# XDzzzzzZyq/b-pinn-kalman-filter

Hardware: AMD Instinct MI355X
Metric: PC-sampler score-net evals/s (NCSN++ 128x128x1, EM + Langevin) (higher is better)
Workload: dtype f32; 1 GPU; configs[2]: NCSN++ 128x128x1 PC sampler, VP-SDE N=1000, euler_maruyama + langevin (snr 0.075), global batch 64 = 64/GPU x 1; model=ncsnpp (62.69M params), global_batch=64, per_gpu_batch=64, parallelism=dp1 (batch-sharded, RCCL), hip_graph=True, pc_graph_allreduce=False

## Files before the change

b-pinn-kalman-filter_amd/csrc/conv_winograd.hip:

```cpp
#include "bpk_common.h"
#include "wino_f24.h"

#include <algorithm>
#include <cstdlib>
#include <type_traits>

namespace {

using f4 = __attribute__((ext_vector_type(4))) float;

constexpr int kTR = 4, kTC = 8;
constexpr int kM = kTR * kTC;
constexpr int kPR = 2 * kTR + 2;
constexpr int kPC = 2 * kTC + 2;
constexpr int kPCp = 24;
constexpr int kCK = 8;
constexpr int kOutRows = 2 * kTR, kOutCols = 2 * kTC;

__device__ inline void wino_filter_range(const float* __restrict__ w, float* __restrict__ U,
                                         int Cin, int Cout, int CoutP, int ft, int64_t first,
                                         int64_t stride) {
  const int64_t total = (int64_t)Cin * CoutP;
  for (int64_t i = first; i < total; i += stride) {
    const int co = (int)(i % CoutP);
    const int ci = (int)(i / CoutP);
    if (co >= Cout) {
      f4* u = reinterpret_cast<f4*>(U + ((int64_t)ci * CoutP + co) * 16);
#pragma unroll
      for (int r = 0; r < 4; ++r) u[r] = f4{0.f, 0.f, 0.f, 0.f};
      continue;
    }
    const float* g = ft ? w + ((int64_t)ci * Cout + co) * 9 : w + ((int64_t)co * Cin + ci) * 9;
    auto gv = [&](int k) { return ft ? g[8 - k] : g[k]; };
    float t[4][3];
#pragma unroll
    for (int c = 0; c < 3; ++c) {
      const float g0 = gv(c), g1 = gv(3 + c), g2 = gv(6 + c);
      t[0][c] = g0;
      t[1][c] = 0.5f * (g0 + g1 + g2);
      t[2][c] = 0.5f * (g0 - g1 + g2);
      t[3][c] = g2;
    }
    float* u = U + ((int64_t)ci * CoutP + co) * 16;
#pragma unroll
    for (int r = 0; r < 4; ++r) {
      const float a0 = t[r][0], a1 = t[r][1], a2 = t[r][2];
      u[4 * r + 0] = a0;
      u[4 * r + 1] = 0.5f * (a0 + a1 + a2);
      u[4 * r + 2] = 0.5f * (a0 - a1 + a2);
      u[4 * r + 3] = a2;
    }
  }
}

__global__ __launch_bounds__(256) void wino_filter_kernel(const float* __restrict__ w,
                                                          float* __restrict__ U, int Cin,
                                                          int Cout, int CoutP, int ft) {
  wino_filter_range(w, U, Cin, Cout, CoutP, ft, (int64_t)blockIdx.x * blockDim.x + threadIdx.x,
                    (int64_t)gridDim.x * blockDim.x);
}

__global__ __launch_bounds__(256) void wino_filter_batch_kernel(const int64_t* __restrict__ jobs) {
  const int64_t* jb = jobs + 6 * (int64_t)blockIdx.y;
  wino_filter_range(reinterpret_cast<const float*>(jb[0]), reinterpret_cast<float*>(jb[1]),
                    (int)jb[2], (int)jb[3], (int)jb[4], (int)jb[5],
                    (int64_t)blockIdx.x * blockDim.x + threadIdx.x,
                    (int64_t)gridDim.x * blockDim.x);
}

__global__ __launch_bounds__(256) void wino_filter24_kernel(const float* __restrict__ w,
                                                            float* __restrict__ U, int Cin,
                                                            int Cout, int CoutP, int ft) {
  const int64_t total = (int64_t)Cin * CoutP;
  for (int64_t i = (int64_t)blockIdx.x * blockDim.x + threadIdx.x; i < total;
       i += (int64_t)gridDim.x * blockDim.x) {
    const int co = (int)(i % CoutP);
    const int ci = (int)(i / CoutP);
    float u[24];
    if (co >= Cout) {
#pragma unroll
      for (int p = 0; p < 24; ++p) u[p] = 0.f;
    } else {
      const float* g = ft ? w + ((int64_t)ci * Cout + co) * 9 : w + ((int64_t)co * Cin + ci) * 9;
      float gg[9];
#pragma unroll
      for (int k = 0; k < 9; ++k) gg[k] = ft ? g[8 - k] : g[k];
      wino24_filter(gg, u);
    }
    f4* dst = reinterpret_cast<f4*>(U) + ((int64_t)ci * (CoutP / 16) + co / 16) * 96 + co % 16;
#pragma unroll
    for (int q = 0; q < 6; ++q)
      dst[16 * q] = f4{u[4 * q], u[4 * q + 1], u[4 * q + 2], u[4 * q + 3]};
  }
}

struct WinoGeo {
  int N, Cin, Cout, H, W;
  int regions_x, regions_y, cout_blocks;
  float div;
  int C1;
  int CoutS;
  int up;
  int ksplit;
  int pair;
};

constexpr int kVS = 20;
constexpr int kPreMaxCin = 1024;


__device__ inline float silu_f(float z) { return z * __builtin_amdgcn_rcpf(1.f + __expf(-z)); }

__device__ inline unsigned udivmod(unsigned a, unsigned d, unsigned& r) {
  if ((d & (d - 1)) == 0) {
    r = a & (d - 1);
    return a >> __builtin_ctz(d);
  }
  const unsigned q = a / d;
  r = a - q * d;
  return q;
}

__device__ inline float div_rn(float a, float b, float r) {
  const float q = a * r;
  return fmaf(fmaf(-q, b, a), r, q);
}

template <int CTRL>
__device__ inline float dpp_f(float v) {
  return __int_as_float(__builtin_amdgcn_mov_dpp(__float_as_int(v), CTRL, 0xF, 0xF, false));
}

__device__ inline void merge_stats(float& m, float& m2, float mo, float m2o, float c) {
  const float d = mo - m;
  m2 = (m2 + m2o) + d * d * (0.5f * c);
  m = 0.5f * (m + mo);
}

#ifdef WINO_TIMING
constexpr unsigned kTsMax = 1u << 17;
__device__ long long g_wino_ts[kTsMax][8];
__device__ unsigned g_wino_cu[kTsMax];
#define WINO_TS_AT(rec, slot)                                                      \
  do {                                                                             \
    if (threadIdx.x == 0 && (rec) < kTsMax) {                                      \
      g_wino_ts[rec][slot] = wall_clock64();                                       \
      if (slot == 0) g_wino_cu[rec] = __smid();                                    \
      if (slot == 0 || slot == 5)                                                  \
        g_wino_ts[rec][6 + slot / 5] = (long long)__builtin_amdgcn_s_memtime();    \
    }                                                                              \
  } while (0)
#else
#define WINO_TS_AT(rec, slot) \
  do {                        \
  } while (0)
#endif
#define WINO_TS(slot) WINO_TS_AT(blockIdx.x, slot)

template <bool PRE, int WG = 4, bool TAIL = false>
__global__ __launch_bounds__(64 * WG, WG == 8 ? 1 : 2) void wino_f23_pipe_kernel(
    const float* __restrict__ x, const float* __restrict__ U, const float* __restrict__ bias,
    const float* __restrict__ skip, const float2* __restrict__ pre, float* __restrict__ y,
    float2* __restrict__ stats, WinoGeo g, int xcd_remap, const float* __restrict__ x2) {
  constexpr int kWN = 16;
  constexpr int kPatch = kCK * kPR * kPCp;
  __shared__ __attribute__((aligned(16))) float s_patch_raw[2][kPatch];
  constexpr int kVBuf = kCK * kM * kVS;
  __shared__ __attribute__((aligned(16))) float s_v[2][kVBuf];
  __shared__ float2 s_ss[PRE ? kPreMaxCin : 1];

  WINO_TS(0);
  const int tid = threadIdx.x;
  const int wave = tid >> 6, lane = tid & 63;
  const unsigned nblk = gridDim.x;
  unsigned b = blockIdx.x;
  if (xcd_remap) b = (b & 7u) * (nblk >> 3) + (b >> 3);
  unsigned cb, rx, ry;
  unsigned r = udivmod(b, (unsigned)g.cout_blocks, cb);
  r = udivmod(r, (unsigned)g.regions_x, rx);
  const int n = (int)udivmod(r, (unsigned)g.regions_y, ry);
  const int oy0 = (int)ry * kOutRows, ox0 = (int)rx * kOutCols;
  const int cout_w = (int)cb * (WG * kWN) + wave * kWN;
  constexpr int kCT = kCK * 4 / WG;
  const int phc = WG == 8 ? __builtin_amdgcn_readfirstlane(tid >> 8) : 0;

  f4 acc[16][2];

  const int64_t plane = (int64_t)g.H * g.W;
  const int C2 = g.Cin - g.C1;
  const float* xn = x + (int64_t)n * g.C1 * plane;
  const float2* pre_n = PRE ? pre + (int64_t)n * g.Cin : nullptr;
  const int kq = lane >> 4, jj = lane & 15;
  const int nch = g.Cin / kCK;

  const __amdgpu_buffer_rsrc_t xrs = __builtin_amdgcn_make_buffer_rsrc(
      const_cast<float*>(xn), 0, (int)(g.C1 * plane * 4), 0x00020000);
  const __amdgpu_buffer_rsrc_t xrs2 = __builtin_amdgcn_make_buffer_rsrc(
      const_cast<float*>(C2 > 0 ? x2 + (int64_t)n * C2 * plane : xn), 0,
      (int)((C2 > 0 ? C2 : g.C1) * plane * 4), 0x00020000);
  const __amdgpu_buffer_rsrc_t urs = __builtin_amdgcn_make_buffer_rsrc(
      const_cast<float*>(U), 0, (int)((int64_t)g.Cin * g.Cout * 64), 0x00020000);

  constexpr int kPos = kPR * kPC;
  int poff, pdst;
  bool pin;
  {
    const int t8 = tid & 255;
    const int t = t8 < kPos ? t8 : 0;
    const int py = t / kPC, px = t - py * kPC;
    const int iy = oy0 - 1 + py, ix = ox0 - 1 + px;
    pin = iy >= 0 && iy < g.H && ix >= 0 && ix < g.W;
    const int cy = min(max(iy, 0), g.H - 1), cx = min(max(ix, 0), g.W - 1);
    poff = (cy * g.W + cx) * 4;
    pdst = py * kPCp + px + phc * kCT * (kPR * kPCp);
  }
  float pv[kCT];
  auto load_patch = [&](int k) {
    const int cc = min(k, nch - 1) * kCK;
    const bool second = cc >= g.C1;
    const int soff = ((second ? cc - g.C1 : cc) + phc * kCT) * (int)plane * 4;
#pragma unroll
    for (int c = 0; c < kCT; ++c)
      pv[c] = __uint_as_float(__builtin_amdgcn_raw_buffer_load_b32(
          second ? xrs2 : xrs, poff, soff + c * (int)plane * 4, 0));
  };
  auto store_patch_from = [&](const float* src, float* sp, int k) {
    const int c0 = min(k, nch - 1) * kCK + phc * kCT;
#pragma unroll
    for (int c = 0; c < kCT; ++c) {
      float v = src[c];
      if (PRE) {
        const float2 st = s_ss[c0 + c];
        v = silu_f(v * st.x + st.y);
      }
      sp[pdst + c * (kPR * kPCp)] = pin ? v : 0.f;
    }
  };
  auto store_patch = [&](float* sp, int k) { store_patch_from(pv, sp, k); };
  f4 uo[2][4];
  const int uoff = ((kq * g.Cout + cout_w + jj) * 16) * 4;
  auto load_u = [&](int ks, int k) {
    const int soff = ((min(k, nch - 1) * kCK + 4 * ks) * g.Cout) * 64;
#pragma unroll
    for (int q = 0; q < 4; ++q) {
      using u4 = __attribute__((ext_vector_type(4))) unsigned;
      const u4 w = __builtin_amdgcn_raw_buffer_load_b128(urs, uoff + q * 16, soff, 0);
      uo[ks][q] = __builtin_bit_cast(f4, w);
    }
  };
  const int tc = (tid & 255) >> 5, tm = tid & 31;
  const int tty = tm / kTC, ttx = tm - tty * kTC;
  float d[4][4];
  auto read_d = [&](const float* sp) {
#pragma unroll
    for (int i = 0; i < 4; ++i)
#pragma unroll
      for (int j = 0; j < 4; j += 2) {
        const float2 v2 =
            *reinterpret_cast<const float2*>(&sp[(tc * kPR + 2 * tty + i) * kPCp + 2 * ttx + j]);
        d[i][j] = v2.x;
        d[i][j + 1] = v2.y;
      }
  };
  auto write_v = [&](float* sv) {
    float t[4][4];
#pragma unroll
    for (int j = 0; j < 4; ++j) {
      t[0][j] = d[0][j] - d[2][j];
      t[1][j] = d[1][j] + d[2][j];
      t[2][j] = d[2][j] - d[1][j];
      t[3][j] = d[1][j] - d[3][j];
    }
    f4* dst = reinterpret_cast<f4*>(&sv[(tc * kM + tm) * kVS]);
#pragma unroll
    for (int i = 0; i < 4; ++i)
      dst[i] = f4{t[i][0] - t[i][2], t[i][1] + t[i][2], t[i][2] - t[i][1], t[i][1] - t[i][3]};
  };

  float pv0[kCT], pv1[kCT];
  load_patch(0);
#pragma unroll
  for (int c = 0; c < kCT; ++c) pv0[c] = pv[c];
  load_patch(1);
#pragma unroll
  for (int c = 0; c < kCT; ++c) pv1[c] = pv[c];
  load_patch(2);
  load_u(0, 0);
  load_u(1, 0);
  if (PRE) {
    for (int c = tid; c < g.Cin; c += 64 * WG) s_ss[c] = pre_n[c];
    __syncthreads();
  }
  WINO_TS(1);
  store_patch_from(pv0, s_patch_raw[0], 0);
  store_patch_from(pv1, s_patch_raw[1], 1);
  __syncthreads();
  WINO_TS(2);
  read_d(s_patch_raw[0]);
  write_v(s_v[0]);
  __syncthreads();

  f4 a[4];
  auto a_src = [&](const float* sv, int grp) {
    const int ks = grp >> 1, mb = grp & 1;
    return reinterpret_cast<const f4*>(&sv[((4 * ks + kq) * kM + mb * 16 + jj) * kVS]);
  };
  {
    const f4* src = a_src(s_v[0], 0);
#pragma unroll
    for (int q = 0; q < 4; ++q) a[q] = src[q];
  }
  auto step = [&](int k, auto sb_c, auto first_c, auto tm_c) __attribute__((always_inline)) {
    constexpr int SB = decltype(sb_c)::value;
    constexpr bool FIRST = decltype(first_c)::value;
    constexpr int TM = decltype(tm_c)::value;
    const float* sv = s_v[SB];
#pragma unroll
    for (int grp = 0; grp < 4; ++grp) {
      const int ks = grp >> 1, mb = grp & 1;
      __builtin_amdgcn_sched_barrier(0);
      if (TM < 3 && grp == 0) read_d(s_patch_raw[SB ^ 1]);
      if (TM < 3 && grp == 1) write_v(s_v[SB ^ 1]);
      if (TM < 2 && grp == 2) store_patch(s_patch_raw[SB], k + 2);
      if (TM < 1 && grp == 3) load_patch(k + 3);
      __builtin_amdgcn_sched_barrier(0);
#pragma unroll
      for (int q = 0; q < 4; ++q) {
#pragma unroll
        for (int pp = 0; pp < 4; ++pp)
          acc[4 * q + pp][mb] = __builtin_amdgcn_mfma_f32_16x16x4f32(
              a[q][pp], uo[ks][q][pp],
              (FIRST && ks == 0) ? f4{0.f, 0.f, 0.f, 0.f} : acc[4 * q + pp][mb], 0, 0, 0);
        if (grp < 3) a[q] = a_src(sv, grp + 1)[q];
        if (TM < 3 && mb == 1) {
          const int soff = ((min(k + 1, nch - 1) * kCK + 4 * ks) * g.Cout) * 64;
          using u4 = __attribute__((ext_vector_type(4))) unsigned;
          const u4 w = __builtin_amdgcn_raw_buffer_load_b128(urs, uoff + q * 16, soff, 0);
          uo[ks][q] = __builtin_bit_cast(f4, w);
        }
      }
    }
    if constexpr (TM < 3) {
      __syncthreads();
      const f4* src = a_src(s_v[SB ^ 1], 0);
#pragma unroll
      for (int q = 0; q < 4; ++q) a[q] = src[q];
    }
  };
  using C0 = std::integral_constant<int, 0>;
  using C1 = std::integral_constant<int, 1>;
  using F = std::false_type;
  WINO_TS(3);
  using T0 = std::integral_constant<int, 0>;
  auto run = [&]() __attribute__((always_inline)) {
    step(0, C0{}, std::true_type{}, T0{});
    int k = 1;
    if constexpr (TAIL) {
      for (; k + 1 <= nch - 4; k += 2) {
        step(k, C1{}, F{}, T0{});
        step(k + 1, C0{}, F{}, T0{});
      }
      step(k, C1{}, F{}, std::integral_constant<int, 1>{});
      step(k + 1, C0{}, F{}, std::integral_constant<int, 2>{});
      step(k + 2, C1{}, F{}, std::integral_constant<int, 3>{});
    } else {
      for (; k + 1 < nch; k += 2) {
        step(k, C1{}, F{}, T0{});
        step(k + 1, C0{}, F{}, T0{});
      }
      if (k < nch) step(k, C1{}, F{}, T0{});
    }
  };
  run();
  WINO_TS(4);

  const float rdiv = 1.f / g.div;
  for (int once = 0; once < 1; ++once) {
    if (cout_w >= g.CoutS) continue;
    const int co = cout_w + jj;
    const float bv = bias ? bias[co] : 0.f;
    const int64_t obase = ((int64_t)n * g.CoutS + co) * plane;
    float lm = 0.f, lm2 = 0.f;
#pragma unroll
    for (int mb = 0; mb < 2; ++mb) {
      const int oy = oy0 + 2 * (2 * mb + (kq >> 1));
      const int ox = ox0 + 8 * (kq & 1);
#pragma unroll
      for (int h = 0; h < 2; ++h) {
#pragma unroll
        for (int e = 0; e < 2; ++e) {
          f4 v;
#pragma unroll
          for (int u = 0; u < 2; ++u) {
            const int rg = 2 * e + u;
            float t[4];
#pragma unroll
            for (int j = 0; j < 4; ++j)
              t[j] = h == 0 ? acc[j][mb][rg] + acc[4 + j][mb][rg] + acc[8 + j][mb][rg]
                            : acc[4 + j][mb][rg] - acc[8 + j][mb][rg] - acc[12 + j][mb][rg];
            v[2 * u] = t[0] + t[1] + t[2] + bv;
            v[2 * u + 1] = t[1] - t[2] - t[3] + bv;
          }
          const int64_t o = obase + (int64_t)(oy + h) * g.W + ox + 4 * e;
          if (skip) {
            const f4 sk = *reinterpret_cast<const f4*>(&skip[o]);
#pragma unroll
            for (int c = 0; c < 4; ++c) v[c] = div_rn(sk[c] + v[c], g.div, rdiv);
          }
          *reinterpret_cast<f4*>(&y[o]) = v;
          if (stats) {
            const float sm = ((v[0] + v[1]) + (v[2] + v[3])) * 0.25f;
            float sm2 = 0.f;
#pragma unroll
            for (int c = 0; c < 4; ++c) sm2 = fmaf(v[c] - sm, v[c] - sm, sm2);
            constexpr float kW[8] = {1.f, 1.f / 2, 1.f / 3, 1.f / 4, 1.f / 5, 1.f / 6, 1.f / 7, 1.f / 8};
            const int st = 4 * mb + 2 * h + e;
            const float d = sm - lm;
            lm = lm + d * kW[st];
            lm2 = (lm2 + sm2) + d * d * (4.f * st * kW[st]);
          }
        }
      }
    }
    if (stats) {
      merge_stats(lm, lm2, __shfl_xor(lm, 16, 64), __shfl_xor(lm2, 16, 64), 32.f);
      merge_stats(lm, lm2, __shfl_xor(lm, 32, 64), __shfl_xor(lm2, 32, 64), 64.f);
      if (kq == 0) {
        const int R = g.regions_x * g.regions_y;
        const int region = (oy0 / kOutRows) * g.regions_x + ox0 / kOutCols;
        stats[((int64_t)n * g.CoutS + co) * R + region] = make_float2(lm, lm2);
      }
    }
  }
  WINO_TS(5);
}

template <bool PRE, bool PAIR>
__device__ __forceinline__ void k16_item(
    unsigned b, const float* __restrict__ x, const float* __restrict__ U,
// ... 208 lines not shown
    const float bv = bias ? bias[co] : 0.f;
    const int oimg = PAIR ? n + (kq & 1) : n;
    const int oxl = PAIR ? 0 : ox0 + 8 * (kq & 1);
    const int64_t obase = ((int64_t)(ks_idx * g.N + oimg) * g.CoutS + co) * plane;
    float lm = 0.f, lm2 = 0.f;
    f4 skv[2][2][2];
    if (skip) {
#pragma unroll
      for (int mb = 0; mb < 2; ++mb)
#pragma unroll
        for (int h = 0; h < 2; ++h)
#pragma unroll
          for (int e = 0; e < 2; ++e)
            skv[mb][h][e] = *reinterpret_cast<const f4*>(
                &skip[obase + (int64_t)(oy0 + 2 * (2 * mb + (kq >> 1)) + h) * g.W + oxl + 4 * e]);
    }
#pragma unroll
    for (int mb = 0; mb < 2; ++mb) {
      const int oy = oy0 + 2 * (2 * mb + (kq >> 1));
      const int ox = oxl;
#pragma unroll
      for (int h = 0; h < 2; ++h) {
#pragma unroll
        for (int e = 0; e < 2; ++e) {
          f4 v;
#pragma unroll
          for (int u = 0; u < 2; ++u) {
            const int rg = 2 * e + u;
            float t[4];
#pragma unroll
            for (int j = 0; j < 4; ++j)
              t[j] = h == 0 ? acc[j][mb][rg] + acc[4 + j][mb][rg] + acc[8 + j][mb][rg]
                            : acc[4 + j][mb][rg] - acc[8 + j][mb][rg] - acc[12 + j][mb][rg];
            v[2 * u] = t[0] + t[1] + t[2] + bv;
            v[2 * u + 1] = t[1] - t[2] - t[3] + bv;
          }
          const int64_t o = obase + (int64_t)(oy + h) * g.W + ox + 4 * e;
          if (skip) {
            const f4 sk = skv[mb][h][e];
#pragma unroll
            for (int c = 0; c < 4; ++c) v[c] = div_rn(sk[c] + v[c], g.div, rdiv);
          }
          *reinterpret_cast<f4*>(&y[o]) = v;
          if (!PAIR && stats) {
            const float sm = ((v[0] + v[1]) + (v[2] + v[3])) * 0.25f;
            float sm2 = 0.f;
#pragma unroll
            for (int c = 0; c < 4; ++c) sm2 = fmaf(v[c] - sm, v[c] - sm, sm2);
            constexpr float kW[8] = {1.f, 1.f / 2, 1.f / 3, 1.f / 4, 1.f / 5, 1.f / 6, 1.f / 7, 1.f / 8};
            const int st = 4 * mb + 2 * h + e;
            const float dd = sm - lm;
            lm = lm + dd * kW[st];
            lm2 = (lm2 + sm2) + dd * dd * (4.f * st * kW[st]);
          }
        }
      }
    }
    if (!PAIR && stats) {
      merge_stats(lm, lm2, __shfl_xor(lm, 16, 64), __shfl_xor(lm2, 16, 64), 32.f);
      merge_stats(lm, lm2, __shfl_xor(lm, 32, 64), __shfl_xor(lm2, 32, 64), 64.f);
      if (kq == 0) {
        const int R = g.regions_x * g.regions_y;
        const int region = (oy0 / kOutRows) * g.regions_x + ox0 / kOutCols;
        stats[((int64_t)n * g.CoutS + co) * R + region] = make_float2(lm, lm2);
      }
    }
  }
  WINO_TS(5);
}

template <bool PRE, bool PAIR = false>
__global__ __launch_bounds__(512, 1) void wino_f23_k16_kernel(
    const float* __restrict__ x, const float* __restrict__ U, const float* __restrict__ bias,
    const float* __restrict__ skip, const float2* __restrict__ pre, float* __restrict__ y,
    float2* __restrict__ stats, WinoGeo g, int xcd_remap, const float* __restrict__ x2,
    unsigned items) {
  const unsigned G = gridDim.x, w = blockIdx.x;
  unsigned first = w, stride = G, end = items;
  if (xcd_remap) {
    const unsigned xc = w & 7u, q = items >> 3, r = items & 7u;
    const unsigned start = xc * q + min(xc, r);
    first = start + (w >> 3);
    stride = G >> 3;
    end = start + q + (xc < r ? 1u : 0u);
  }
  for (unsigned b = first; b < end; b += stride) {
    if (b != first) __syncthreads();
    k16_item<PRE, PAIR>(b, x, U, bias, skip, pre, y, stats, g, x2);
  }
}

constexpr int kM24 = 16;
constexpr int kVS24 = 28;

struct Item24Carry {
  f4 uo[2][6];
  int tab_n;
  bool u_ready;
};

template <bool PRE, bool TAILK>
__device__ __forceinline__ void k16_item24(
    unsigned b, unsigned nb, const float* __restrict__ x, const float* __restrict__ U,
    const float* __restrict__ bias, const float* __restrict__ skip,
    const float2* __restrict__ pre, float* __restrict__ y, float2* __restrict__ stats,
    const WinoGeo& g, const float* __restrict__ x2, Item24Carry& carry) {
  constexpr int kOob = (int)0x80000000u;
  constexpr int CK = 16;
  constexpr int kPatch = CK * kPR * kPCp;
  __shared__ __attribute__((aligned(16))) float s_patch_raw[2][kPatch];
  constexpr int kVBuf = CK * kM24 * kVS24;
  __shared__ __attribute__((aligned(16))) float s_v[2][kVBuf];
  __shared__ float2 s_ss[PRE ? kPreMaxCin : 1];

  const int tid = threadIdx.x;
  const int wave = tid >> 6, lane = tid & 63;
  unsigned cb, rx, ry;
  unsigned r = udivmod(b, (unsigned)g.cout_blocks, cb);
  r = udivmod(r, (unsigned)g.regions_x, rx);
  r = udivmod(r, (unsigned)g.regions_y, ry);
  unsigned nn;
  const int ks_idx = (int)udivmod(r, (unsigned)g.N, nn);
  const int n = (int)nn;
  const int oy0 = (int)ry * kOutRows, ox0 = (int)rx * kOutCols;
  const int cout_w = (int)cb * 128 + wave * 16;
  const int ph = __builtin_amdgcn_readfirstlane(tid >> 8);
  WINO_TS_AT(b, 0);
  bool u_next = false;
  if (TAILK && nb != ~0u) {
    unsigned cb2, t2;
    unsigned r2 = udivmod(nb, (unsigned)g.cout_blocks, cb2);
    r2 = udivmod(r2, (unsigned)g.regions_x, t2);
    r2 = udivmod(r2, (unsigned)g.regions_y, t2);
    u_next = cb2 == cb && (int)udivmod(r2, (unsigned)g.N, t2) == ks_idx;
  }

  f4 acc[24];
  const int64_t plane = (int64_t)g.H * g.W;
  const int up = g.up;
  const int64_t xplane = plane >> (2 * up);
  const int C2 = g.Cin - g.C1;
  const float* xn = x + (int64_t)n * g.C1 * xplane;
  const float2* pre_n = PRE ? pre + (int64_t)n * g.Cin : nullptr;
  const int kq = lane >> 4, jj = lane & 15;
  const int nch = g.Cin / CK / max(g.ksplit, 1);
  const int kb = ks_idx * nch;

  const __amdgpu_buffer_rsrc_t xrs = __builtin_amdgcn_make_buffer_rsrc(
      const_cast<float*>(xn), 0, (int)(g.C1 * xplane * 4), 0x00020000);
  const __amdgpu_buffer_rsrc_t xrs2 = __builtin_amdgcn_make_buffer_rsrc(
      const_cast<float*>(C2 > 0 ? x2 + (int64_t)n * C2 * plane : xn), 0,
      (int)((C2 > 0 ? C2 : g.C1) * plane * 4), 0x00020000);
  const __amdgpu_buffer_rsrc_t urs = __builtin_amdgcn_make_buffer_rsrc(
      const_cast<float*>(U), 0, (int)((int64_t)g.Cin * g.Cout * 96), 0x00020000);

  constexpr int kPos = kPR * kPC;
  int poff, pdst;
  bool pin;
  {
    const int t8 = tid & 255;
    const int t = t8 < kPos ? t8 : 0;
    const int py = t / kPC, px = t - py * kPC;
    const int iy = oy0 - 1 + py, ix = ox0 - 1 + px;
    pin = iy >= 0 && iy < g.H && ix >= 0 && ix < g.W;
    const int cy = min(max(iy, 0), g.H - 1), cx = min(max(ix, 0), g.W - 1);
    poff = ((cy >> up) * (g.W >> up) + (cx >> up)) * 4;
    pdst = py * kPCp + px + ph * 8 * (kPR * kPCp);
  }
  float pv[8];
  auto load_patch_part = [&](float* dst, int k, int c0, int cn, bool guard = false) {
    const int cc = (kb + min(k, nch - 1)) * CK;
    const bool second = cc >= g.C1;
    const int soff = ((second ? cc - g.C1 : cc) + ph * 8) * (int)xplane * 4;
    const int po = (guard && k >= nch) ? kOob : poff;
#pragma unroll
    for (int c = c0; c < c0 + cn; ++c)
      dst[c] = __uint_as_float(__builtin_amdgcn_raw_buffer_load_b32(
          second ? xrs2 : xrs, po, soff + c * (int)xplane * 4, 0));
  };
  auto store_patch_part = [&](const float* src, float* sp, int k, int c0, int cn) {
    const int cb0 = (kb + min(k, nch - 1)) * CK + ph * 8;
#pragma unroll
    for (int c = c0; c < c0 + cn; ++c) {
      float v = src[c];
      if (PRE) {
        const float2 st = s_ss[cb0 + c];
        v = silu_f(v * st.x + st.y);
      }
      sp[pdst + c * (kPR * kPCp)] = pin ? v : 0.f;
    }
  };
  f4(&uo)[2][6] = carry.uo;
  const int uoff = ((kq * g.Cout + cout_w) * 24 + jj * 4) * 4;
  auto u_soff = [&](int k, int ks) {
    return (((kb + min(k, nch - 1)) * CK + 4 * ks) * g.Cout) * 96;
  };
  const int u_soff0[2] = {__builtin_amdgcn_readfirstlane(u_soff(0, 0)),
                          __builtin_amdgcn_readfirstlane(u_soff(0, 1))};
  auto load_u = [&](int slot, int k, int ks) {
    const int soff = u_soff(k, ks);
#pragma unroll
    for (int q = 0; q < 6; ++q)
      uo[slot][q] = __builtin_bit_cast(
          f4, __builtin_amdgcn_raw_buffer_load_b128(urs, uoff + q * 256, soff, 0));
  };
  const int th = __builtin_amdgcn_readfirstlane(wave & 1);
  const int tc = 4 * kq + (wave >> 1);
  const int tty = jj >> 2, ttx = jj & 3;
  float d[3][6];
  auto read_d = [&](const float* sp) {
#pragma unroll
    for (int i = 0; i < 3; ++i) {
      const float* row = &sp[(tc * kPR + 2 * tty + th + i) * kPCp + 4 * ttx];
      const f4 v4 = *reinterpret_cast<const f4*>(row);
      const float2 v2 = *reinterpret_cast<const float2*>(row + 4);
      d[i][0] = v4[0];
      d[i][1] = v4[1];
      d[i][2] = v4[2];
      d[i][3] = v4[3];
      d[i][4] = v2.x;
      d[i][5] = v2.y;
    }
  };
  auto write_v = [&](float* sv) {
    float rx_[6], ry_[6], vx[6], vy[6];
#pragma unroll
    for (int j = 0; j < 6; ++j) wino24_data_rows(d[0][j], d[1][j], d[2][j], th, rx_[j], ry_[j]);
    wino24_data_cols(rx_, vx);
    wino24_data_cols(ry_, vy);
    f4* dst = reinterpret_cast<f4*>(&sv[(tc * kM24 + jj) * kVS24 + 12 * th]);
    dst[0] = f4{vx[0], vx[1], vx[2], vx[3]};
    dst[1] = f4{vx[4], vx[5], vy[0], vy[1]};
    dst[2] = f4{vy[2], vy[3], vy[4], vy[5]};
  };

  const bool tab_load = PRE && carry.tab_n != n;
  const bool u_have = TAILK && carry.u_ready;
  carry.tab_n = n;
  carry.u_ready = u_next;
  {
    float pv0[8], pv1[8];
    float2 tv[kPreMaxCin / 512];
    if (tab_load) {
#pragma unroll
      for (int i = 0; i < kPreMaxCin / 512; ++i) tv[i] = pre_n[min(tid + 512 * i, g.Cin - 1)];
    }
    __builtin_amdgcn_sched_barrier(0);
    load_patch_part(pv0, 0, 0, 8);
    __builtin_amdgcn_sched_barrier(0);
    load_patch_part(pv1, 1, 0, 8, TAILK);
    load_patch_part(pv, 2, 0, 8, TAILK);
    if (!u_have) {
      load_u(0, 0, 0);
      load_u(1, 0, 1);
    }
    __builtin_amdgcn_sched_barrier(0);
    if (tab_load) {
#pragma unroll
      for (int i = 0; i < kPreMaxCin / 512; ++i)
        if (tid + 512 * i < g.Cin) s_ss[tid + 512 * i] = tv[i];
      __syncthreads();
    }
    store_patch_part(pv0, s_patch_raw[0], 0, 0, 8);
    __syncthreads();
    read_d(s_patch_raw[0]);
    write_v(s_v[0]);
    if (!TAILK || nch > 1) store_patch_part(pv1, s_patch_raw[1], 1, 0, 8);
  }
  __syncthreads();
  WINO_TS_AT(b, 1);

  f4 a[4];
  auto a_src = [&](const float* sv, int ks) {
    return reinterpret_cast<const f4*>(&sv[((4 * ks + kq) * kM24 + jj) * kVS24]);
  };
  {
    const f4* src = a_src(s_v[0], 0);
#pragma unroll
    for (int q = 0; q < 4; ++q) a[q] = src[q];
  }
  auto step = [&](int k, auto sb_c, auto first_c, auto tail_c) __attribute__((always_inline)) {
    constexpr int SB = decltype(sb_c)::value;
    constexpr bool FIRST = decltype(first_c)::value;
    constexpr int TL = decltype(tail_c)::value;
    const float* sv = s_v[SB];
#pragma unroll
    for (int grp = 0; grp < 8; ++grp) {
      const int ks = grp >> 1, hf = grp & 1;
      __builtin_amdgcn_sched_barrier(0);
      if (grp == 0 && TL < 3) read_d(s_patch_raw[SB ^ 1]);
      if (grp == 1 && TL < 3) write_v(s_v[SB ^ 1]);
      if (grp == 2 && TL < 2) store_patch_part(pv, s_patch_raw[SB], k + 2, 0, 4);
      if (grp == 3 && TL < 2) store_patch_part(pv, s_patch_raw[SB], k + 2, 4, 4);
      if (grp == 4 && TL < 1) load_patch_part(pv, k + 3, 0, 4);
      if (grp == 5 && TL < 1) load_patch_part(pv, k + 3, 4, 4);
      __builtin_amdgcn_sched_barrier(0);
#pragma unroll
      for (int qq = 0; qq < 3; ++qq) {
        const int q = 3 * hf + qq;
        const int fi = 6 * ks + q;
#pragma unroll
        for (int pp = 0; pp < 4; ++pp)
          acc[4 * q + pp] = __builtin_amdgcn_mfma_f32_16x16x4f32(
              a[fi & 3][pp], uo[ks & 1][q][pp],
              (FIRST && ks == 0) ? f4{0.f, 0.f, 0.f, 0.f} : acc[4 * q + pp], 0, 0, 0);
        if (fi + 4 < 24) a[fi & 3] = a_src(sv, (fi + 4) / 6)[(fi + 4) % 6];
        if (ks < 2 || TL < 3 || TAILK) {
          const int soff = ks < 2 ? u_soff(k, ks + 2)
                                  : (TL < 3 ? u_soff(k + 1, ks - 2) : u_soff0[ks - 2]);
          uo[ks & 1][q] = __builtin_bit_cast(
              f4, __builtin_amdgcn_raw_buffer_load_b128(urs, uoff + q * 256, soff, 0));
        }
      }
    }
    if (TL < 3) {
      __syncthreads();
      const f4* src = a_src(s_v[SB ^ 1], 0);
#pragma unroll
      for (int q = 0; q < 4; ++q) a[q] = src[q];
    }
  };
  using C0 = std::integral_constant<int, 0>;
  using C1 = std::integral_constant<int, 1>;
  using T2 = std::integral_constant<int, 2>;
  using T3 = std::integral_constant<int, 3>;
  using Fi = std::true_type;
  using No = std::false_type;
  WINO_TS_AT(b, 2);
  if (!TAILK) {
    step(0, C0{}, Fi{}, C0{});
    int k = 1;
    for (; k + 1 < nch; k += 2) {
      step(k, C1{}, No{}, C0{});
      step(k + 1, C0{}, No{}, C0{});
    }
    if (k < nch) step(k, C1{}, No{}, C0{});
  } else {
    if (nch >= 4) {
      step(0, C0{}, Fi{}, C0{});
      int k = 1;
      for (; k + 3 < nch; k += 2) {
        step(k, C1{}, No{}, C0{});
        step(k + 1, C0{}, No{}, C0{});
      }
    } else {
#pragma unroll
      for (int i = 0; i < 24; ++i) acc[i] = f4{0.f, 0.f, 0.f, 0.f};
    }
    if (nch >= 4) step(nch - 3, C1{}, No{}, C1{});
    step(nch - 2, C0{}, No{}, T2{});
    step(nch - 1, C1{}, No{}, T3{});
  }
  WINO_TS_AT(b, 3);

  const float rdiv = 1.f / g.div;
  if (cout_w < g.CoutS) {
    const int co = cout_w + jj;
    const float bv = bias ? bias[co] : 0.f;
    const int64_t obase = ((int64_t)(ks_idx * g.N + n) * g.CoutS + co) * plane +
                          (int64_t)(oy0 + 2 * kq) * g.W + ox0;
    float lm = 0.f, lm2 = 0.f;
    f4 skv[2][4];
    if (skip) {
#pragma unroll
      for (int h = 0; h < 2; ++h)
#pragma unroll
        for (int rg = 0; rg < 4; ++rg)
          skv[h][rg] = *reinterpret_cast<const f4*>(&skip[obase + (int64_t)h * g.W + 4 * rg]);
    }
#pragma unroll
    for (int h = 0; h < 2; ++h) {
#pragma unroll
      for (int rg = 0; rg < 4; ++rg) {
        float t[6], yv[4];
#pragma unroll
        for (int j = 0; j < 6; ++j)
          t[j] = wino24_out_rows(acc[j][rg], acc[6 + j][rg], acc[12 + j][rg], acc[18 + j][rg], h);
        wino24_out_cols(t, yv);
        f4 v = f4{yv[0] + bv, yv[1] + bv, yv[2] + bv, yv[3] + bv};
        const int64_t o = obase + (int64_t)h * g.W + 4 * rg;
        if (skip) {
          const f4 sk = skv[h][rg];
#pragma unroll
          for (int c = 0; c < 4; ++c) v[c] = div_rn(sk[c] + v[c], g.div, rdiv);
        }
        *reinterpret_cast<f4*>(&y[o]) = v;
        if (stats) {
          const float sm = ((v[0] + v[1]) + (v[2] + v[3])) * 0.25f;
          float sm2 = 0.f;
#pragma unroll
          for (int c = 0; c < 4; ++c) sm2 = fmaf(v[c] - sm, v[c] - sm, sm2);
          constexpr float kW[8] = {1.f, 1.f / 2, 1.f / 3, 1.f / 4, 1.f / 5, 1.f / 6, 1.f / 7, 1.f / 8};
          const int st = 4 * h + rg;
          const float dd = sm - lm;
          lm = lm + dd * kW[st];
          lm2 = (lm2 + sm2) + dd * dd * (4.f * st * kW[st]);
        }
      }
    }
    WINO_TS_AT(b, 4);
    if (stats) {
      merge_stats(lm, lm2, __shfl_xor(lm, 16, 64), __shfl_xor(lm2, 16, 64), 32.f);
      merge_stats(lm, lm2, __shfl_xor(lm, 32, 64), __shfl_xor(lm2, 32, 64), 64.f);
      if (kq == 0) {
        const int R = g.regions_x * g.regions_y;
        const int region = (oy0 / kOutRows) * g.regions_x + ox0 / kOutCols;
        stats[((int64_t)n * g.CoutS + co) * R + region] = make_float2(lm, lm2);
      }
    }
  }
  WINO_TS_AT(b, 5);
}

template <bool PRE, bool TAILK>
__global__ __launch_bounds__(512, 1) void wino_f24_k16_kernel(
    const float* __restrict__ x, const float* __restrict__ U, const float* __restrict__ bias,
    const float* __restrict__ skip, const float2* __restrict__ pre, float* __restrict__ y,
    float2* __restrict__ stats, WinoGeo g, int xcd_remap, const float* __restrict__ x2,
    unsigned items) {
  const unsigned G = gridDim.x, w = blockIdx.x;
  unsigned first = w, stride = G, end = items;
  if (xcd_remap) {
    const unsigned xc = w & 7u, q = items >> 3, r = items & 7u;
    const unsigned start = xc * q + min(xc, r);
    first = start + (w >> 3);
    stride = G >> 3;
    end = start + q + (xc < r ? 1u : 0u);
  }
  Item24Carry carry;
  carry.tab_n = -1;
  carry.u_ready = false;
  for (unsigned b = first; b < end; b += stride) {
    if (b != first) __syncthreads();
    const unsigned nb = b + stride < end ? b + stride : ~0u;
    k16_item24<PRE, TAILK>(b, nb, x, U, bias, skip, pre, y, stats, g, x2, carry);
  }
}

__global__ __launch_bounds__(256) void wino_splitk_reduce_kernel(
    const float* __restrict__ part, int S, const float* __restrict__ bias,
    const float* __restrict__ skip, float* __restrict__ y, float2* __restrict__ stats,
    WinoGeo g) {
  const int lane = threadIdx.x & 63;
  const int q = threadIdx.x;
  unsigned b = blockIdx.x, reg, cg;
  const unsigned R = (unsigned)(g.regions_x * g.regions_y);
  unsigned r = udivmod(b, R, reg);
  int n = (int)udivmod(r, (unsigned)(g.CoutS / 8), cg);
  const int co = (int)cg * 8 + (q >> 5);
  const int rem = q & 31;
  const int row = rem >> 2;
  int c4 = rem & 3;
  if (g.pair) {
    n = 2 * n + (c4 >> 1);
    c4 &= 1;
  }
  const int oy0 = (int)(reg / g.regions_x) * kOutRows, ox0 = (int)(reg % g.regions_x) * kOutCols;
  const int64_t plane = (int64_t)g.H * g.W;
  const int64_t slab = (int64_t)g.N * g.CoutS * plane;
  const int64_t o = ((int64_t)n * g.CoutS + co) * plane + (int64_t)(oy0 + row) * g.W + ox0 + 4 * c4;
  f4 v = *reinterpret_cast<const f4*>(&part[o]);
  for (int s = 1; s < S; ++s) v += *reinterpret_cast<const f4*>(&part[s * slab + o]);
  const float bv = bias ? bias[co] : 0.f;
  v += f4{bv, bv, bv, bv};
  if (skip) {
    const f4 sk = *reinterpret_cast<const f4*>(&skip[o]);
    const float rdiv = 1.f / g.div;
#pragma unroll
    for (int c = 0; c < 4; ++c) v[c] = div_rn(sk[c] + v[c], g.div, rdiv);
  }
  *reinterpret_cast<f4*>(&y[o]) = v;
  if (!stats || g.pair) return;
  float mm = ((v[0] + v[1]) + (v[2] + v[3])) * 0.25f;
  float qq = 0.f;
#pragma unroll
  for (int e = 0; e < 4; ++e) qq = fmaf(v[e] - mm, v[e] - mm, qq);
  merge_stats(mm, qq, dpp_f<0xB1>(mm), dpp_f<0xB1>(qq), 4.f);
  merge_stats(mm, qq, dpp_f<0x4E>(mm), dpp_f<0x4E>(qq), 8.f);
  merge_stats(mm, qq, dpp_f<0x141>(mm), dpp_f<0x141>(qq), 16.f);
  merge_stats(mm, qq, dpp_f<0x140>(mm), dpp_f<0x140>(qq), 32.f);
  merge_stats(mm, qq, __shfl_xor(mm, 16, 64), __shfl_xor(qq, 16, 64), 64.f);
  if ((lane & 31) == 0) stats[((int64_t)n * g.CoutS + co) * R + reg] = make_float2(mm, qq);
}

}

static int cout_padded(int Cout) { return (Cout + 63) / 64 * 64; }

static int cu_count() {
  static const int cus = [] {
    int dev = 0, n = 0;
    (void)hipGetDevice(&dev);
    (void)hipDeviceGetAttribute(&n, hipDeviceAttributeMultiprocessorCount, dev);
    return n > 0 ? n : 256;
  }();
  return cus;
}


extern "C" int64_t bpk_conv3x3_wino_filter_bytes(int Cin, int Cout) {
  return (int64_t)16 * Cin * cout_padded(Cout) * (int64_t)sizeof(float);
}

extern "C" int64_t bpk_conv3x3_wino_filter24_bytes(int Cin, int Cout) {
  return (int64_t)24 * Cin * cout_padded(Cout) * (int64_t)sizeof(float);
}

using FilterKernel = void (*)(const float*, float*, int, int, int, int);

static int wino_filter(FilterKernel kern, const float* weight, float* U, int Cin, int Cout,
                       int ft, void* stream) {
  BPK_REQUIRE(Cin > 0 && Cout > 0, "conv3x3_wino_filter: bad channels %d -> %d", Cin, Cout);
  const int64_t total = (int64_t)Cin * cout_padded(Cout);
  hipLaunchKernelGGL(kern, dim3((unsigned)std::min<int64_t>(bpk::ceil_div(total, 256), 4096)),
                     dim3(256), 0, bpk::as_stream(stream), weight, U, Cin, Cout,
                     cout_padded(Cout), ft);
  BPK_LAUNCH_CHECK("conv3x3_wino_filter");
  return BPK_OK;
}

extern "C" int bpk_conv3x3_wino_filter_f32(const float* weight, float* U, int Cin, int Cout,
                                           void* stream) {
  return wino_filter(wino_filter_kernel, weight, U, Cin, Cout, 0, stream);
}

extern "C" int bpk_conv3x3_wino_filter_ft_f32(const float* weight, float* U, int Cin, int Cout,
                                              void* stream) {
  return wino_filter(wino_filter_kernel, weight, U, Cin, Cout, 1, stream);
}

extern "C" int bpk_conv3x3_wino_filter24_f32(const float* weight, float* U, int Cin, int Cout,
                                             void* stream) {
  return wino_filter(wino_filter24_kernel, weight, U, Cin, Cout, 0, stream);
}

extern "C" int bpk_conv3x3_wino_filter24_ft_f32(const float* weight, float* U, int Cin, int Cout,
                                                void* stream) {
  return wino_filter(wino_filter24_kernel, weight, U, Cin, Cout, 1, stream);
}

extern "C" int bpk_conv3x3_wino_filter_batch_f32(const int64_t* jobs, int n, int max_elems,
                                                 void* stream) {
  BPK_REQUIRE(n >= 0 && n < 65536 && max_elems >= 0, "conv3x3_wino_filter_batch: bad job count");
  if (n == 0 || max_elems == 0) return BPK_OK;
  BPK_REQUIRE(jobs != nullptr, "conv3x3_wino_filter_batch: jobs is NULL");
  const dim3 grid((unsigned)std::min<int64_t>(bpk::ceil_div(max_elems, 256), 64), (unsigned)n);
  hipLaunchKernelGGL(wino_filter_batch_kernel, grid, dim3(256), 0, bpk::as_stream(stream), jobs);
  BPK_LAUNCH_CHECK("conv3x3_wino_filter_batch");
  return BPK_OK;
}


extern "C" int bpk_conv3x3_wino_supported(int N, int Cin, int Cout, int H, int W) {
  return N > 0 && Cin > 0 && Cin % kCK == 0 && Cout % 16 == 0 && H % kOutRows == 0 &&
         W % kOutCols == 0;
}

static bool k16_channels_ok(int Cin, int C1, int Cout) {
  return Cin % 16 == 0 && C1 % 16 == 0 && cout_padded(Cout) % 128 == 0;
}

static bool wino_pair_ok(int N, int Cin, int Cout, int H, int W) {
  return N > 0 && N % 2 == 0 && W == 8 && H > 0 && H % kOutRows == 0 && Cout % 16 == 0 &&
         k16_channels_ok(Cin, Cin, Cout);
}

extern "C" int bpk_conv3x3_wino_pair_supported(int N, int Cin, int Cout, int H, int W) {
  return wino_pair_ok(N, Cin, Cout, H, W);
}

extern "C" int bpk_conv3x3_wino_up2_supported(int N, int Cin, int Cout, int H, int W) {
  return bpk_conv3x3_wino_supported(N, Cin, Cout, H, W) && k16_channels_ok(Cin, Cin, Cout);
}

extern "C" int bpk_conv3x3_wino_f24_supported(int N, int Cin, int C1, int Cout, int H, int W) {
  return N > 0 && Cin > 0 && Cin <= kPreMaxCin && C1 > 0 && C1 <= Cin && Cout > 0 &&
         Cout % 16 == 0 && k16_channels_ok(Cin, C1, Cout) && H > 0 && H % kOutRows == 0 && W > 0 &&
         W % kOutCols == 0;
}


struct WinoArgs {
  const float *x, *x2, *pre, *U, *bias, *skip;
  float *y, *stats;
  void* stream;
};

static WinoGeo k16_geo(int N, int Cin, int C1, int Cout, int H, int W, float div, int up, int S,
                       int pair) {
  const int CoutP = cout_padded(Cout);
  WinoGeo g{};
  g.N = N, g.Cin = Cin, g.C1 = C1, g.Cout = CoutP, g.CoutS = Cout, g.H = H, g.W = W;
  g.regions_x = pair ? 1 : W / kOutCols;
  g.regions_y = H / kOutRows;
  g.cout_blocks = CoutP / 128;
  g.div = div, g.up = up, g.ksplit = S, g.pair = pair;
  return g;
}

static int64_t k16_items(const WinoGeo& g) {
  return (int64_t)(g.pair ? g.N / 2 : g.N) * g.regions_x * g.regions_y * g.cout_blocks * g.ksplit;
}

using K16Kernel = void (*)(const float*, const float*, const float*, const float*, const float2*,
                           float*, float2*, WinoGeo, int, const float*, unsigned);

static int k16_launch(bool f24, const WinoGeo& g, const WinoArgs& a) {
  const int64_t items = k16_items(g);
  BPK_REQUIRE(items < (1LL << 31), "conv3x3_wino: grid too large");
  static const K16Kernel kKern[2][2][2] = {
      {{wino_f23_k16_kernel<false, false>, wino_f23_k16_kernel<false, true>},
       {wino_f23_k16_kernel<true, false>, wino_f23_k16_kernel<true, true>}},
      {{wino_f24_k16_kernel<false, false>, wino_f24_k16_kernel<false, true>},
       {wino_f24_k16_kernel<true, false>, wino_f24_k16_kernel<true, true>}}};
  const bool even = (g.Cin / 16 / g.ksplit) % 2 == 0;
  const unsigned grid = (unsigned)std::min<int64_t>(items, cu_count());
  const bool raw = g.ksplit > 1;
  hipLaunchKernelGGL(kKern[f24][a.pre != nullptr][f24 ? even : g.pair != 0], dim3(grid), dim3(512),
                     0, bpk::as_stream(a.stream), a.x, a.U, raw ? nullptr : a.bias,
                     raw ? nullptr : a.skip, reinterpret_cast<const float2*>(a.pre), a.y,
                     raw ? nullptr : reinterpret_cast<float2*>(a.stats), g, grid % 8 == 0 ? 1 : 0,
                     a.x2, (unsigned)items);
  BPK_LAUNCH_CHECK(f24 ? "conv3x3_wino_f24" : "conv3x3_wino_k16");
  return BPK_OK;
}

static int wino_f24_check(int N, int Cin, int C1, int Cout, int H, int W) {
  BPK_REQUIRE(bpk_conv3x3_wino_f24_supported(N, Cin, C1, Cout, H, W),
              "conv3x3_wino_f24: unsupported shape N=%d Cin=%d (C1=%d) Cout=%d H=%d W=%d (need "
              "Cin, C1 %% 16, Cout %% 128, H %% 8, W %% 16 == 0, Cin <= %d)", N, Cin, C1, Cout, H,
              W, kPreMaxCin);
  return BPK_OK;
}

static int wino_pair_check(const WinoArgs& a, int N, int Cin, int Cout, int H, int W) {
  BPK_REQUIRE(!a.x2 && !a.stats, "conv3x3_wino pair form (W == 8): one source, no statistics");
  BPK_REQUIRE(wino_pair_ok(N, Cin, Cout, H, W),
              "conv3x3_wino pair form: unsupported shape N=%d Cin=%d Cout=%d H=%d W=%d (need "
              "W == 8, N even, H %% 8, Cin %% 16, Cout %% 128 == 0)", N, Cin, Cout, H, W);
  BPK_REQUIRE(!a.pre || 2 * Cin <= kPreMaxCin, "conv3x3_wino pair form: GroupNorm prologue over "
              "%d > %d channels", Cin, kPreMaxCin / 2);
  return BPK_OK;
}

using PipeKernel = void (*)(const float*, const float*, const float*, const float*, const float2*,
                            float*, float2*, WinoGeo, int, const float*);

static int wino_ex(const WinoArgs& a, int C1, float div, int N, int Cin, int Cout, int H, int W) {
  if (!a.x2) C1 = Cin;
  if (W == 8) {
    const int rc = wino_pair_check(a, N, Cin, Cout, H, W);
    return rc != BPK_OK ? rc : k16_launch(false, k16_geo(N, Cin, Cin, Cout, H, W, div, 0, 1, 1), a);
  }
  BPK_REQUIRE(C1 > 0 && C1 <= Cin && C1 % kCK == 0,
              "conv3x3_wino: bad channel split C1=%d of Cin=%d", C1, Cin);
  BPK_REQUIRE(bpk_conv3x3_wino_supported(N, Cin, Cout, H, W),
              "conv3x3_wino: unsupported shape N=%d Cin=%d Cout=%d H=%d W=%d (need Cin %% 8, "
              "Cout %% 16, H %% 8, W %% 16 == 0)", N, Cin, Cout, H, W);
  BPK_REQUIRE(!a.pre || Cin <= kPreMaxCin,
              "conv3x3_wino: GroupNorm prologue over %d > %d input channels (the table in LDS): "
              "apply it to the input first", Cin, kPreMaxCin);
  if (k16_channels_ok(Cin, C1, Cout))
    return k16_launch(false, k16_geo(N, Cin, C1, Cout, H, W, div, 0, 1, 0), a);
  const int CoutP = cout_padded(Cout);
  const bool wg8 = a.pre && !a.skip && CoutP % 128 == 0;
  WinoGeo g{};
  g.N = N, g.Cin = Cin, g.C1 = C1, g.Cout = CoutP, g.CoutS = Cout, g.H = H, g.W = W;
  g.regions_x = W / kOutCols, g.regions_y = H / kOutRows, g.cout_blocks = CoutP / (wg8 ? 128 : 64);
  g.div = div;
  const int64_t blocks = (int64_t)N * g.regions_x * g.regions_y * g.cout_blocks;
  BPK_REQUIRE(blocks < (1LL << 31), "conv3x3_wino: grid too large");
  const int nch = Cin / kCK;
  const bool tail = a.pre && nch % 2 == 0 && nch >= 4;
  static const PipeKernel kPipe[2][2][2] = {
      {{wino_f23_pipe_kernel<false, 4, false>, wino_f23_pipe_kernel<false, 4, false>},
       {wino_f23_pipe_kernel<false, 8, false>, wino_f23_pipe_kernel<false, 8, false>}},
      {{wino_f23_pipe_kernel<true, 4, false>, wino_f23_pipe_kernel<true, 4, true>},
       {wino_f23_pipe_kernel<true, 8, false>, wino_f23_pipe_kernel<true, 8, true>}}};
  hipLaunchKernelGGL(kPipe[a.pre != nullptr][wg8][tail], dim3((unsigned)blocks),
                     dim3(wg8 ? 512 : 256), 0, bpk::as_stream(a.stream), a.x, a.U, a.bias, a.skip,
                     reinterpret_cast<const float2*>(a.pre), a.y,
                     reinterpret_cast<float2*>(a.stats), g, blocks % 8 == 0 ? 1 : 0, a.x2);
  BPK_LAUNCH_CHECK("conv3x3_wino_pipe");
  return BPK_OK;
}

extern "C" int bpk_conv3x3_wino_ex_f32(const float* x, const float* x2, int C1, const float* pre,
                                       const float* U, const float* bias, const float* skip,
                                       float div, float* y, float* stats, int N, int Cin,
                                       int Cout, int H, int W, void* stream) {
  return wino_ex({x, x2, pre, U, bias, skip, y, stats, stream}, C1, div, N, Cin, Cout, H, W);
}

extern "C" int bpk_conv3x3_wino_pre_f32(const float* x, const float* pre, const float* U,
                                        const float* bias, const float* skip, float div, float* y,
                                        int N, int Cin, int Cout, int H, int W, void* stream) {
  return wino_ex({x, nullptr, pre, U, bias, skip, y, nullptr, stream}, Cin, div, N, Cin, Cout, H,
                 W);
}

extern "C" int bpk_conv3x3_wino_residual_f32(const float* x, const float* U, const float* bias,
                                             const float* skip, float div, float* y, int N,
                                             int Cin, int Cout, int H, int W, void* stream) {
  return bpk_conv3x3_wino_pre_f32(x, nullptr, U, bias, skip, div, y, N, Cin, Cout, H, W, stream);
}

extern "C" int bpk_conv3x3_wino_f32(const float* x, const float* U, const float* bias, float* y,
                                    int N, int Cin, int Cout, int H, int W, void* stream) {
  return bpk_conv3x3_wino_pre_f32(x, nullptr, U, bias, nullptr, 1.0f, y, N, Cin, Cout, H, W,
                                  stream);
// ... 95 lines not shown
```

Baseline: 827.3 score-net evals/s.

## Transpose MFMA operands in Winograd F24 k16 epilogue to change output lane mapping

Swaps the A/B operands of the 16x16x4 MFMA so the accumulator layout puts output channels across lanes differently, then rewrites the epilogue to index by four channels per lane with per-row spatial tiles, loading bias as a vector and computing per-channel stats via quad DPP transposes plus shuffles. The aim is to change the store and skip-load access pattern and the stats reduction cost. It relies on new lane variables (tty, ttx) and changes which channel each lane writes, so correctness depends on the rest of the kernel defining them consistently. It also adds an optional debug macro path that collapses the stores into one.

Measured after the change: 853.9 score-net evals/s, median of 6. +3.2%, better.

```diff
diff --git a/b-pinn-kalman-filter_amd/csrc/conv_winograd.hip b/b-pinn-kalman-filter_amd/csrc/conv_winograd.hip
--- a/b-pinn-kalman-filter_amd/csrc/conv_winograd.hip
+++ b/b-pinn-kalman-filter_amd/csrc/conv_winograd.hip
@@ -135,6 +135,19 @@
   const float d = mo - m;
   m2 = (m2 + m2o) + d * d * (0.5f * c);
   m = 0.5f * (m + mo);
+}
+
+template <int CTRL>
+__device__ inline void quad_swap(float& lo, float& hi, bool upper) {
+  const float plo = dpp_f<CTRL>(lo), phi = dpp_f<CTRL>(hi);
+  lo = upper ? phi : lo;
+  hi = upper ? hi : plo;
+}
+__device__ inline void quad_transpose(float (&a)[4], int t) {
+  quad_swap<0xB1>(a[0], a[1], t & 1);
+  quad_swap<0xB1>(a[2], a[3], t & 1);
+  quad_swap<0x4E>(a[0], a[2], t & 2);
+  quad_swap<0x4E>(a[1], a[3], t & 2);
 }
 
 #ifdef WINO_TIMING
@@ -949,7 +962,7 @@
 #pragma unroll
         for (int pp = 0; pp < 4; ++pp)
           acc[4 * q + pp] = __builtin_amdgcn_mfma_f32_16x16x4f32(
-              a[fi & 3][pp], uo[ks & 1][q][pp],
+              uo[ks & 1][q][pp], a[fi & 3][pp],
               (FIRST && ks == 0) ? f4{0.f, 0.f, 0.f, 0.f} : acc[4 * q + pp], 0, 0, 0);
         if (fi + 4 < 24) a[fi & 3] = a_src(sv, (fi + 4) / 6)[(fi + 4) % 6];
         if (ks < 2 || TL < 3 || TAILK) {
@@ -1002,57 +1015,80 @@
 
   const float rdiv = 1.f / g.div;
   if (cout_w < g.CoutS) {
-    const int co = cout_w + jj;
-    const float bv = bias ? bias[co] : 0.f;
-    const int64_t obase = ((int64_t)(ks_idx * g.N + n) * g.CoutS + co) * plane +
-                          (int64_t)(oy0 + 2 * kq) * g.W + ox0;
-    float lm = 0.f, lm2 = 0.f;
-    f4 skv[2][4];
+    const int co0 = cout_w + 4 * kq;
+    f4 bv = f4{0.f, 0.f, 0.f, 0.f};
+    if (bias) bv = f4{bias[co0], bias[co0 + 1], bias[co0 + 2], bias[co0 + 3]};
+    const int64_t obase = ((int64_t)(ks_idx * g.N + n) * g.CoutS + co0) * plane +
+                          (int64_t)(oy0 + 2 * tty) * g.W + ox0 + 4 * ttx;
+    float sm[2][4], sm2[2][4];
+    f4 skv[4][2];
     if (skip) {
 #pragma unroll
-      for (int h = 0; h < 2; ++h)
-#pragma unroll
-        for (int rg = 0; rg < 4; ++rg)
-          skv[h][rg] = *reinterpret_cast<const f4*>(&skip[obase + (int64_t)h * g.W + 4 * rg]);
-    }
-#pragma unroll
-    for (int h = 0; h < 2; ++h) {
-#pragma unroll
-      for (int rg = 0; rg < 4; ++rg) {
+      for (int r = 0; r < 4; ++r)
+#pragma unroll
+        for (int h = 0; h < 2; ++h)
+#ifdef WINO_F24_EPI_ONE_STORE
+          skv[r][h] = f4{0.f, 0.f, 0.f, 0.f};
+#else
+          skv[r][h] = *reinterpret_cast<const f4*>(&skip[obase + r * plane + (int64_t)h * g.W]);
+#endif
+    }
+#ifdef WINO_F24_EPI_ONE_STORE
+    f4 vsum = f4{0.f, 0.f, 0.f, 0.f};
+#endif
+#pragma unroll
+    for (int r = 0; r < 4; ++r) {
+#pragma unroll
+      for (int h = 0; h < 2; ++h) {
         float t[6], yv[4];
 #pragma unroll
         for (int j = 0; j < 6; ++j)
-          t[j] = wino24_out_rows(acc[j][rg], acc[6 + j][rg], acc[12 + j][rg], acc[18 + j][rg], h);
+          t[j] = wino24_out_rows(acc[j][r], acc[6 + j][r], acc[12 + j][r], acc[18 + j][r], h);
         wino24_out_cols(t, yv);
-        f4 v = f4{yv[0] + bv, yv[1] + bv, yv[2] + bv, yv[3] + bv};
-        const int64_t o = obase + (int64_t)h * g.W + 4 * rg;
+        f4 v = f4{yv[0] + bv[r], yv[1] + bv[r], yv[2] + bv[r], yv[3] + bv[r]};
         if (skip) {
-          const f4 sk = skv[h][rg];
+          const f4 sk = skv[r][h];
 #pragma unroll
           for (int c = 0; c < 4; ++c) v[c] = div_rn(sk[c] + v[c], g.div, rdiv);
         }
-        *reinterpret_cast<f4*>(&y[o]) = v;
+#ifdef WINO_F24_EPI_ONE_STORE
+        vsum += v;
+#else
+        *reinterpret_cast<f4*>(&y[obase + r * plane + (int64_t)h * g.W]) = v;
+#endif
         if (stats) {
-          const float sm = ((v[0] + v[1]) + (v[2] + v[3])) * 0.25f;
-          float sm2 = 0.f;
-#pragma unroll
-          for (int c = 0; c < 4; ++c) sm2 = fmaf(v[c] - sm, v[c] - sm, sm2);
-          constexpr float kW[8] = {1.f, 1.f / 2, 1.f / 3, 1.f / 4, 1.f / 5, 1.f / 6, 1.f / 7, 1.f / 8};
-          const int st = 4 * h + rg;
-          const float dd = sm - lm;
-          lm = lm + dd * kW[st];
-          lm2 = (lm2 + sm2) + dd * dd * (4.f * st * kW[st]);
+          const float m = ((v[0] + v[1]) + (v[2] + v[3])) * 0.25f;
+          float q = 0.f;
+#pragma unroll
+          for (int c = 0; c < 4; ++c) q = fmaf(v[c] - m, v[c] - m, q);
+          sm[h][r] = m, sm2[h][r] = q;
         }
       }
     }
+#ifdef WINO_F24_EPI_ONE_STORE
+    *reinterpret_cast<f4*>(&y[obase]) = vsum;
+#endif
     WINO_TS_AT(b, 4);
     if (stats) {
-      merge_stats(lm, lm2, __shfl_xor(lm, 16, 64), __shfl_xor(lm2, 16, 64), 32.f);
-      merge_stats(lm, lm2, __shfl_xor(lm, 32, 64), __shfl_xor(lm2, 32, 64), 64.f);
-      if (kq == 0) {
+#pragma unroll
+      for (int h = 0; h < 2; ++h) {
+        quad_transpose(sm[h], ttx);
+        quad_transpose(sm2[h], ttx);
+      }
+      constexpr float kW[8] = {1.f, 1.f / 2, 1.f / 3, 1.f / 4, 1.f / 5, 1.f / 6, 1.f / 7, 1.f / 8};
+      float lm = 0.f, lm2 = 0.f;
+#pragma unroll
+      for (int st = 0; st < 8; ++st) {
+        const float dd = sm[st >> 2][st & 3] - lm;
+        lm = lm + dd * kW[st];
+        lm2 = (lm2 + sm2[st >> 2][st & 3]) + dd * dd * (4.f * st * kW[st]);
+      }
+      merge_stats(lm, lm2, __shfl_xor(lm, 4, 64), __shfl_xor(lm2, 4, 64), 32.f);
+      merge_stats(lm, lm2, __shfl_xor(lm, 8, 64), __shfl_xor(lm2, 8, 64), 64.f);
+      if (tty == 0) {
         const int R = g.regions_x * g.regions_y;
         const int region = (oy0 / kOutRows) * g.regions_x + ox0 / kOutCols;
-        stats[((int64_t)n * g.CoutS + co) * R + region] = make_float2(lm, lm2);
+        stats[((int64_t)n * g.CoutS + co0 + ttx) * R + region] = make_float2(lm, lm2);
       }
     }
   }
```
